# 1pathplanningzzj/pointnet_refine

Hardware: AMD Instinct MI355X
Metric: lane segments/sec (fwd+bwd) at B=4096,N=1024; HBM GB/s vs roofline (higher is better)
Workload: dtype f32 (large GEMMs: 2xfp16-split MFMA, 3 products, fp32 accumulate); 1 GPU; LineRefineNet training step (fwd + deep-supervision L1 + bwd + Adam), B=4096/GPU, N=1024, M=32, C=4; global_batch=4096, points=1024, parallelism=dp1, decoder_chunk=4096

## Files before the change

pointnet_refine_amd/csrc/prh_gemm_h2.hpp:

```cpp
#pragma once
#include "prh_gemm_s3.hpp"

namespace prh {

constexpr int H2_BK = 32;
constexpr int H2_PLANE = 256 * H2_BK * 2;
constexpr int H2_OPER = 2 * H2_PLANE;
constexpr int H2_STAGE = 2 * H2_OPER;
constexpr int H2_LDS = 2 * H2_STAGE;

__device__ __forceinline__ int h2_off(int row, int k) {
  return row * 64 + ((((k >> 3) ^ (-(row >> 2))) & 3) << 4) + ((k & 7) << 1);
}

inline size_t h2_weight_bytes(int N, int K) {
  return S3_WHDR + (size_t)((N + 255) / 256) * ((K + H2_BK - 1) / H2_BK) * H2_OPER;
}

__global__ __launch_bounds__(256) void prep_weights_h2_kernel(const float* __restrict__ W, int N,
                                                              int K, long ldw, char* __restrict__ out,
                                                              const float* __restrict__ amax) {
  const int KT = (K + H2_BK - 1) / H2_BK;
  const int NT_ = (N + 255) / 256;
  const long total = (long)NT_ * 256 * KT * 4;
  const long i = (long)blockIdx.x * blockDim.x + threadIdx.x;
  if (i >= total) return;
  const int chunk = (int)(i & 3);
  long t = i >> 2;
  const int k_tile = (int)(t % KT); t /= KT;
  const int row = (int)(t & 255);
  const int n_tile = (int)(t >> 8);
  const int n = n_tile * 256 + row;
  const float S = pow2_scale(load_amax(amax));
  float v[8];
#pragma unroll
  for (int j = 0; j < 8; ++j) {
    const int k = k_tile * H2_BK + chunk * 8 + j;
    v[j] = (n < N && k < K) ? W[(size_t)n * ldw + k] * S : 0.f;
  }
  uint4 h, l;
  split2h(v[0], v[1], h.x, l.x);
  split2h(v[2], v[3], h.y, l.y);
  split2h(v[4], v[5], h.z, l.z);
  split2h(v[6], v[7], h.w, l.w);
  char* base = out + ((size_t)n_tile * KT + k_tile) * H2_OPER + h2_off(row, chunk * 8);
  *reinterpret_cast<uint4*>(base) = h;
  *reinterpret_cast<uint4*>(base + H2_PLANE) = l;
}

template <int I0 = 0, int I1 = 8>
__device__ __forceinline__ void h2_compute(f32x4 (&acc)[8][4], const char* st, int wm, int wn, int l15,
                                           int kc) {
  f16x8 wh[4], wl[4];
#pragma unroll
  for (int j = 0; j < 4; ++j) {
    const char* q = st + H2_OPER + h2_off(wn + j * 16 + l15, kc * 8);
    wh[j] = *reinterpret_cast<const f16x8*>(q);
    wl[j] = *reinterpret_cast<const f16x8*>(q + H2_PLANE);
  }
#pragma unroll
  for (int i = I0; i < I1; ++i) {
    const char* q = st + h2_off(wm + i * 16 + l15, kc * 8);
    const f16x8 ah = *reinterpret_cast<const f16x8*>(q);
    const f16x8 al = *reinterpret_cast<const f16x8*>(q + H2_PLANE);
#pragma unroll
    for (int j = 0; j < 4; ++j) {
      acc[i][j] = __builtin_amdgcn_mfma_f32_16x16x32_f16(al, wh[j], acc[i][j], 0, 0, 0);
      acc[i][j] = __builtin_amdgcn_mfma_f32_16x16x32_f16(ah, wl[j], acc[i][j], 0, 0, 0);
      acc[i][j] = __builtin_amdgcn_mfma_f32_16x16x32_f16(ah, wh[j], acc[i][j], 0, 0, 0);
    }
  }
}

template <int PRO, int EPI, bool PP = false>
__global__ __launch_bounds__(512, 2) void gemm_nt_h2_kernel(const NTParams p,
                                                            const char* __restrict__ Wp) {
  static_assert(PRO == PRO_NONE || PRO == PRO_BNRELU || PRO == PRO_GATE1, "prologue not supported");
  extern __shared__ __attribute__((aligned(16))) char smem[];
#ifdef PRH_STAMP
  unsigned t_acc[4] = {0u, 0u, 0u, 0u};
  unsigned long long t_prev = __builtin_amdgcn_s_memtime();
#endif
  const int tid = threadIdx.x, lane = tid & 63, wave = tid >> 6;
  const int l15 = lane & 15, kc = lane >> 4;
  const int wm = (wave >> 2) * 128, wn = (wave & 3) * 64;
  const int vb = xcd_remap(blockIdx.x, gridDim.x);
  const int tile_n = vb % p.tiles_n, tile_m = vb / p.tiles_n;
  const int m0 = tile_m * 256, n0 = tile_n * 256;
  const int KT = (p.K + H2_BK - 1) / H2_BK;

  const int sc = (tid & 7) * 4;
  const int sr = tid >> 3;
  const int KP = (KT + 2) * H2_BK;
  float* coef = reinterpret_cast<float*>(smem + H2_LDS);
  const float sA = pow2_scale(load_amax(p.amaxA));
  const float unscale = 1.f / (sA * pow2_scale(load_amax(p.amaxW)));

  f32x4 acc[8][4];
#pragma unroll
  for (int i = 0; i < 8; ++i)
#pragma unroll
    for (int j = 0; j < 4; ++j)
#pragma unroll
      for (int r = 0; r < 4; ++r) acc[i][j][r] = 0.f;

  float4 ra[2][4];
  const char* wsrc = Wp + (size_t)tile_n * KT * H2_OPER + tid * 16;
  const unsigned lds0 = (unsigned)(unsigned long)((__attribute__((address_space(3))) char*)smem);
  const unsigned wdst = __builtin_amdgcn_readfirstlane(lds0 + H2_OPER + wave * 1024);
  auto dma_w = [&](int kt, int stage) {
    const char* q = wsrc + (size_t)(kt < KT ? kt : KT - 1) * H2_OPER;
#pragma unroll
    for (int pc = 0; pc < 4; ++pc) glds16(q + pc * 8192, wdst + stage * H2_STAGE + pc * 8192);
  };
  constexpr int NA = PRO == PRO_GATE1 ? 0 : 4;
  int arows = p.M - m0; arows = arows > 256 ? 256 : arows;
  const __amdgpu_buffer_rsrc_t rsA = __builtin_amdgcn_make_buffer_rsrc(
      (void*)(p.A + (size_t)m0 * p.lda), 0,
      PRO == PRO_GATE1 ? 0 : (int)(((size_t)(arows - 1) * p.lda + p.K) * 4), 0x00020000);
  int voA[4];
  float gi[4] = {0.f, 0.f, 0.f, 0.f};
#pragma unroll
  for (int j = 0; j < 4; ++j) {
    voA[j] = ((sr + 64 * j) * (int)p.lda + sc) * 4;
    if (PRO == PRO_GATE1) {
      const int row = m0 + sr + 64 * j;
      gi[j] = row < p.M ? p.A[(size_t)row * p.lda] : 0.f;
    }
  }
  auto load_tile = [&](int kt, float4 (&r)[4]) {
    if (PRO == PRO_GATE1) return;
    const int so = kt * (H2_BK * 4);
#pragma unroll
    for (int j = 0; j < 4; ++j)
      r[j] = __builtin_bit_cast(float4, __builtin_amdgcn_raw_buffer_load_b128(rsA, voA[j] + so, 0, 0));
  };
  auto store_tile = [&](int kt, char* st, const float4 (&r_)[4]) {
    const int k = kt * H2_BK + sc;
    const bool kok = k < p.K || PRO != PRO_NONE;
    float4 ka = zero4(), kb = zero4();
    if (PRO != PRO_NONE) {
      ka = *reinterpret_cast<const float4*>(coef + k);
      kb = *reinterpret_cast<const float4*>(coef + KP + k);
    }
#pragma unroll
    for (int j = 0; j < 4; ++j) {
      const int r = sr + 64 * j;
      float4 v;
      if (PRO == PRO_GATE1) v = pro_apply<PRO>(make_float4(gi[j], 0.f, 0.f, 0.f), zero4(), ka, kb, zero4());
      else v = pro_apply<PRO>(r_[j], zero4(), ka, kb, zero4());
      v.x = kok ? v.x : 0.f; v.y = kok ? v.y : 0.f; v.z = kok ? v.z : 0.f; v.w = kok ? v.w : 0.f;
      if (PRO == PRO_NONE) { v.x *= sA; v.y *= sA; v.z *= sA; v.w *= sA; }
      uint2 h, l;
      split2h(v.x, v.y, h.x, l.x);
      split2h(v.z, v.w, h.y, l.y);
      char* q = st + h2_off(r, sc);
      *reinterpret_cast<uint2*>(q) = h;
      *reinterpret_cast<uint2*>(q + H2_PLANE) = l;
    }
  };
  auto iter = [&](int kt, auto cs, auto tail) {
    constexpr int CS = decltype(cs)::value;
    constexpr bool TAIL = decltype(tail)::value;
    char* cur = smem + (kt & 1) * H2_STAGE;
    char* nxt = smem + ((kt + 1) & 1) * H2_STAGE;
    if (PRO != PRO_GATE1) {
#pragma unroll
      for (int j = 0; j < 4; ++j)
        asm volatile("" : "+v"(ra[CS][j].x), "+v"(ra[CS][j].y), "+v"(ra[CS][j].z), "+v"(ra[CS][j].w));
      __builtin_amdgcn_sched_barrier(0);
    }
    dma_w(kt + 1, (kt + 1) & 1);
    __builtin_amdgcn_sched_barrier(0);
    if (!TAIL) load_tile(kt + 2, ra[CS ^ 1]);
    __builtin_amdgcn_sched_barrier(0);
    h2_compute<0, 8>(acc, cur, wm, wn, l15, kc);
    store_tile(kt + 1, nxt, ra[CS]);
#pragma unroll
    for (int g = 0; g < 48; ++g) {
      __builtin_amdgcn_sched_group_barrier(0x008, 2, 0);
      __builtin_amdgcn_sched_group_barrier(0x002, 3, 0);
    }
    if (TAIL) asm volatile("s_waitcnt vmcnt(0)" ::: "memory");
    else asm volatile("s_waitcnt vmcnt(%0)" ::"i"(NA) : "memory");
    __syncthreads();
  };

  dma_w(0, 0);
  __builtin_amdgcn_sched_barrier(0);
  load_tile(0, ra[0]);
  load_tile(1, ra[1]);
  if (PRO != PRO_NONE) {
    for (int i = tid; i < KP; i += 512) {
      const bool in = i < p.K;
      coef[i] = in ? p.pa[i] * sA : 0.f;
      coef[KP + i] = in ? p.pb[i] * sA : 0.f;
    }
    __syncthreads();
  }
  store_tile(0, smem, ra[0]);
  asm volatile("s_waitcnt vmcnt(0)" ::: "memory");
  __syncthreads();
  PRH_TICK(0)
  int kt = 0;
  if constexpr (!PP) {
    for (; kt + 2 < KT; kt += 2) {
      iter(kt, std::integral_constant<int, 1>{}, std::false_type{});
      iter(kt + 1, std::integral_constant<int, 0>{}, std::false_type{});
    }
    if (kt < KT) iter(kt, std::integral_constant<int, 1>{}, std::true_type{});
    if (kt + 1 < KT) iter(kt + 1, std::integral_constant<int, 0>{}, std::true_type{});
  } else {
    const int wr = __builtin_amdgcn_readfirstlane(wave >> 2);
    const int aoff = h2_off(wm + l15, kc * 8);
    const int woff = H2_OPER + h2_off(wn + l15, kc * 8);
    f16x8 wh[4], wl[4], ah[2], al[2];
    auto store_pass = [&](int kt1, char* st, const float4& r_, const int j) {
      const int k = kt1 * H2_BK + sc;
      const bool kok = k < p.K || PRO != PRO_NONE;
      float4 ka = zero4(), kb = zero4();
      if (PRO != PRO_NONE) {
        ka = *reinterpret_cast<const float4*>(coef + k);
        kb = *reinterpret_cast<const float4*>(coef + KP + k);
      }
      float4 v;
      if (PRO == PRO_GATE1) v = pro_apply<PRO>(make_float4(gi[j], 0.f, 0.f, 0.f), zero4(), ka, kb, zero4());
      else v = pro_apply<PRO>(r_, zero4(), ka, kb, zero4());
      v.x = kok ? v.x : 0.f; v.y = kok ? v.y : 0.f; v.z = kok ? v.z : 0.f; v.w = kok ? v.w : 0.f;
      if (PRO == PRO_NONE) { v.x *= sA; v.y *= sA; v.z *= sA; v.w *= sA; }
      uint2 h, l;
      split2h(v.x, v.y, h.x, l.x);
      split2h(v.z, v.w, h.y, l.y);
      char* q = st + h2_off(sr + 64 * j, sc);
      *reinterpret_cast<uint2*>(q) = h;
      *reinterpret_cast<uint2*>(q + H2_PLANE) = l;
    };
    auto phase = [&](int kt_, auto mp, auto cs, auto tail) {
      constexpr int MP = decltype(mp)::value;
      constexpr int CS = decltype(cs)::value;
      constexpr bool TAIL = decltype(tail)::value;
      const char* cur = smem + (kt_ & 1) * H2_STAGE;
      char* nxt = smem + ((kt_ + 1) & 1) * H2_STAGE;
      __builtin_amdgcn_sched_barrier(0);
      if (MP == 0) {
#pragma unroll
        for (int j = 0; j < 4; ++j) {
          wh[j] = *reinterpret_cast<const f16x8*>(cur + woff + j * 1024);
          wl[j] = *reinterpret_cast<const f16x8*>(cur + woff + j * 1024 + H2_PLANE);
        }
      }
#pragma unroll
      for (int i = 0; i < 2; ++i) {
        ah[i] = *reinterpret_cast<const f16x8*>(cur + aoff + (2 * MP + i) * 1024);
        al[i] = *reinterpret_cast<const f16x8*>(cur + aoff + (2 * MP + i) * 1024 + H2_PLANE);
      }
      __builtin_amdgcn_sched_barrier(0);
      store_pass(kt_ + 1, nxt, ra[CS][MP], MP);
      __builtin_amdgcn_sched_barrier(0);
      if (MP == 0) dma_w(kt_ + 1, (kt_ + 1) & 1);
      __builtin_amdgcn_sched_barrier(0);
      if (!TAIL && PRO != PRO_GATE1)
        ra[CS ^ 1][MP] = __builtin_bit_cast(float4, __builtin_amdgcn_raw_buffer_load_b128(rsA, voA[MP] + (kt_ + 2) * (H2_BK * 4), 0, 0));
      __builtin_amdgcn_sched_barrier(0);
      if (MP == 3) {
        if (TAIL || PRO == PRO_GATE1) asm volatile("s_waitcnt vmcnt(0)" ::: "memory");
        else asm volatile("s_waitcnt vmcnt(4)" ::: "memory");
      }
      asm volatile("s_waitcnt lgkmcnt(0)" ::: "memory");
      __builtin_amdgcn_sched_barrier(0);
      __builtin_amdgcn_s_barrier();
      __builtin_amdgcn_sched_barrier(0);
      __builtin_amdgcn_s_setprio(1);
#pragma unroll
      for (int i = 0; i < 2; ++i)
#pragma unroll
        for (int j = 0; j < 4; ++j)
          acc[2 * MP + i][j] = __builtin_amdgcn_mfma_f32_16x16x32_f16(al[i], wh[j], acc[2 * MP + i][j], 0, 0, 0);
#pragma unroll
      for (int i = 0; i < 2; ++i)
#pragma unroll
        for (int j = 0; j < 4; ++j)
          acc[2 * MP + i][j] = __builtin_amdgcn_mfma_f32_16x16x32_f16(ah[i], wl[j], acc[2 * MP + i][j], 0, 0, 0);
#pragma unroll
      for (int i = 0; i < 2; ++i)
#pragma unroll
        for (int j = 0; j < 4; ++j)
          acc[2 * MP + i][j] = __builtin_amdgcn_mfma_f32_16x16x32_f16(ah[i], wh[j], acc[2 * MP + i][j], 0, 0, 0);
      __builtin_amdgcn_s_setprio(0);
      __builtin_amdgcn_sched_barrier(0);
      __builtin_amdgcn_s_barrier();
      __builtin_amdgcn_sched_barrier(0);
    };
    auto tile = [&](int kt_, auto cs, auto tail) {
      phase(kt_, std::integral_constant<int, 0>{}, cs, tail);
      phase(kt_, std::integral_constant<int, 1>{}, cs, tail);
      phase(kt_, std::integral_constant<int, 2>{}, cs, tail);
      phase(kt_, std::integral_constant<int, 3>{}, cs, tail);
    };
    if (wr == 1) __builtin_amdgcn_s_barrier();
    for (; kt + 2 < KT; kt += 2) {
      tile(kt, std::integral_constant<int, 1>{}, std::false_type{});
      tile(kt + 1, std::integral_constant<int, 0>{}, std::false_type{});
    }
    if (kt < KT) tile(kt, std::integral_constant<int, 1>{}, std::true_type{});
    if (kt + 1 < KT) tile(kt + 1, std::integral_constant<int, 0>{}, std::true_type{});
    if (wr == 0) __builtin_amdgcn_s_barrier();
  }
  asm volatile("s_waitcnt vmcnt(0)" ::: "memory");
  __syncthreads();
  PRH_TICK(1)
#pragma unroll
  for (int i = 0; i < 8; ++i)
#pragma unroll
    for (int j = 0; j < 4; ++j)
#pragma unroll
      for (int r = 0; r < 4; ++r) acc[i][j][r] *= unscale;
  nt_epilogue_vec<EPI, 4>(acc, p, m0 + wm, n0 + wn, tile_m * 2 + (wave >> 2), lane,
                          reinterpret_cast<float*>(smem) + wave * (32 * EPI_LDW));
#ifdef PRH_STAMP
  PRH_TICK(2)
  asm volatile("s_waitcnt vmcnt(0)" ::: "memory");
  PRH_TICK(3)
  const int which = (p.K == 1024 && p.N == 1984) ? 0 : (p.K == 1984 && p.N == 1024) ? 1 : (p.K == 256 && p.N == 1536) ? 2 : (p.K == 512 && p.N == 1024) ? 3 : -1;
  if (g_prh_stamp != nullptr && which >= 0 && blockIdx.x == gridDim.x / 2 + 3 && lane == 0 && (wave & 3) == 0) {
    unsigned* o = g_prh_stamp + 64 + which * 16 + (wave >> 2) * 8;
#pragma unroll
    for (int i = 0; i < 4; ++i) o[i] = t_acc[i];
    o[4] = (unsigned)KT;
  }
#endif
}

typedef __fp16 fp16x4 __attribute__((__vector_size__(4 * sizeof(__fp16))));
constexpr int TR_ROW = 576;
constexpr int TR_PLANE = 16 * TR_ROW;
constexpr int TR_OPER = 2 * TR_PLANE;
constexpr int TR_STAGE = 2 * TR_OPER;
constexpr int TR_LDS = 2 * TR_STAGE;

__device__ __forceinline__ f16x8 tr_fragment(const char* plane, int col0, int lane) {
  const int g = lane >> 4, j = lane & 15;
  const char* a = plane + ((g >> 1) * 8 + (j >> 2)) * TR_ROW + (col0 + (g & 1) * 16 + 4 * (j & 3)) * 2;
  const fp16x4 lo = __builtin_amdgcn_ds_read_tr16_b64_v4f16(
      (__attribute__((address_space(3))) fp16x4*)(a));
  const fp16x4 hi = __builtin_amdgcn_ds_read_tr16_b64_v4f16(
      (__attribute__((address_space(3))) fp16x4*)(a + 4 * TR_ROW));
  struct Pair { fp16x4 a, b; } pr = {lo, hi};
  return __builtin_bit_cast(f16x8, pr);
}

constexpr int TR_PACE = 8;
constexpr int TR_PACE_SPINS = 256;
constexpr int TR_SIDE_MAX_COLS = 4096;
inline size_t tr_side_lds(int cols) { return (size_t)3 * ((cols + 255) / 256 * 256) * 4 + 64; }
typedef unsigned int u32x4 __attribute__((ext_vector_type(4)));

template <int PROB, bool SIDE = false>
__global__ __launch_bounds__(512, 2) void gemm_tn_tr_kernel(const TNParams p) {
  static_assert(PROB == PRO_NONE || PROB == PRO_BNRELU, "prologue not supported");
  extern __shared__ __attribute__((aligned(16))) char smem[];
  const int tid = threadIdx.x, lane = tid & 63, wave = tid >> 6;
  const int wm = (wave >> 2) * 128, wn = (wave & 3) * 64;
  int b = xcd_remap(blockIdx.x, gridDim.x);
  const int tile_n = b % p.tiles_n; b /= p.tiles_n;
  const int tile_m = b % p.tiles_m; b /= p.tiles_m;
  const int split = b;
  const int m0 = tile_m * 256, n0 = tile_n * 256;
  const int p_begin = split * p.rows_per_split;
  int p_end = p_begin + p.rows_per_split;
  if (p_end > p.P) p_end = p.P;
  const int KT = (p_end - p_begin + S3_BK - 1) / S3_BK;

  const int c4 = (tid & 63) * 4, r8 = tid >> 6;
  const bool aok = (m0 + c4) < p.Mo, bok = (n0 + c4) < p.Ni;
  const float sA = pow2_scale(load_amax(p.amaxA)), sB = pow2_scale(load_amax(p.amaxB));
  const float sAm = aok ? sA : 0.f, sBm = bok ? sB : 0.f;
  float4 qa = zero4(), qb = zero4();
  if (PROB == PRO_BNRELU && bok) {
    qa = ldg4(p.qa + n0 + c4); qb = ldg4(p.qb + n0 + c4);
    qa.x *= sB; qa.y *= sB; qa.z *= sB; qa.w *= sB; qb.x *= sB; qb.y *= sB; qb.z *= sB; qb.w *= sB;
  }
  const bool want_cs = p.colsum != nullptr && tile_n == 0;

  f32x16 acc[4][2];
#pragma unroll
  for (int i = 0; i < 4; ++i)
#pragma unroll
    for (int j = 0; j < 2; ++j)
#pragma unroll
      for (int r = 0; r < 16; ++r) acc[i][j][r] = 0.f;

  const int nrows = p_end - p_begin > 0 ? p_end - p_begin : 0;
  int acols = p.Mo - m0; acols = acols > 256 ? 256 : acols;
  int bcols = p.Ni - n0; bcols = bcols > 256 ? 256 : bcols;
  const size_t abytes = nrows > 0 ? ((size_t)(nrows - 1) * p.lda + acols) * 4 : 0;
  const size_t bbytes = nrows > 0 ? ((size_t)(nrows - 1) * p.ldb + bcols) * 4 : 0;
  const __amdgpu_buffer_rsrc_t rsA = __builtin_amdgcn_make_buffer_rsrc(
      (void*)(p.A + (size_t)p_begin * p.lda + m0), 0, (int)abytes, 0x00020000);
  const __amdgpu_buffer_rsrc_t rsB = __builtin_amdgcn_make_buffer_rsrc(
      (void*)(p.B + (size_t)p_begin * p.ldb + n0), 0, (int)bbytes, 0x00020000);
  const int stepA = (int)p.lda * 4, stepB = (int)p.ldb * 4;
  const int voA = r8 * stepA + c4 * 4, voB = r8 * stepB + c4 * 4;

  float4 va[2][2], vb[2][2];
  float4 cs = zero4();
  auto load_tile = [&](int kt, float4 (&xa)[2], float4 (&xb)[2]) {
    const int oa = voA + kt * S3_BK * stepA, ob = voB + kt * S3_BK * stepB;
#pragma unroll
    for (int j = 0; j < 2; ++j) {
      xa[j] = __builtin_bit_cast(float4, __builtin_amdgcn_raw_buffer_load_b128(rsA, oa + j * 8 * stepA, 0, 0));
      xb[j] = __builtin_bit_cast(float4, __builtin_amdgcn_raw_buffer_load_b128(rsB, ob + j * 8 * stepB, 0, 0));
    }
  };
// ... 212 lines not shown
```

pointnet_refine_amd/csrc/prh_lib.hip:

```cpp
#include "../../include/pointnet_refine_hip.h"

#include <hip/hip_runtime.h>
#include <stdarg.h>
#include <stdio.h>
#include <string.h>

#include <mutex>
#include <vector>

#include <stdlib.h>

#include "prh_gemm.hpp"
#include "prh_attn.hpp"
#include "prh_attn16.hpp"
#include "prh_gemm_s3.hpp"
#include "prh_gemm_h2.hpp"
#include "prh_b16.hpp"
#include "prh_small.hpp"
#include "prh_attnfold.hpp"
#include "prh_fused.hpp"
#include "prh_context.hpp"
#include "prh_metrics.hpp"
#include "prh_drive.hpp"
#include "prh_match.hpp"
#include "prh_bev.hpp"
#include "prh_view.hpp"
#include "prh_fuse.hpp"
#include "prh_pcd.hpp"
#include "prh_kernels.hpp"

using namespace prh;

namespace {

thread_local char g_err[512] = "";

int fail(int code, const char* fmt, ...) {
  va_list ap;
  va_start(ap, fmt);
  vsnprintf(g_err, sizeof(g_err), fmt, ap);
  va_end(ap);
  return code;
}

#define HIP_TRY(expr)                                                                  \
  do {                                                                                 \
    hipError_t e_ = (expr);                                                            \
    if (e_ != hipSuccess)                                                              \
      return fail(PRH_ERR_HIP, "%s failed: %s (%s:%d)", #expr, hipGetErrorString(e_),  \
                  __FILE__, __LINE__);                                                 \
  } while (0)

#define LAUNCH_CHECK() HIP_TRY(hipGetLastError())
#define TRY_RC(x)                  \
  do {                             \
    int rc_ = (x);                 \
    if (rc_ != PRH_OK) return rc_; \
  } while (0)
#ifndef PRH_GEMM_DEFAULT
#define PRH_GEMM_DEFAULT 3
#endif

struct ProfRec { hipEvent_t e0, e1; char name[64]; double flops, bytes; };
struct Profiler {
  std::mutex mu;
  std::vector<ProfRec> recs;
  size_t used = 0;
  bool on = false;
} g_prof;

struct ProfScope {
  ProfRec* r = nullptr; hipStream_t st;
  ProfScope(const char* name, double flops, double bytes, hipStream_t s) : st(s) {
    if (!g_prof.on) return;
    std::lock_guard<std::mutex> lk(g_prof.mu);
    if (g_prof.used >= g_prof.recs.size()) return;
    r = &g_prof.recs[g_prof.used++];
    snprintf(r->name, sizeof(r->name), "%s", name);
    r->flops = flops; r->bytes = bytes;
    (void)hipEventRecord(r->e0, st);
  }
  ~ProfScope() { if (r) (void)hipEventRecord(r->e1, st); }
};

inline size_t align_up(size_t x, size_t a) { return (x + a - 1) / a * a; }
inline int cdiv(long a, long b) { return (int)((a + b - 1) / b); }

struct Arena {
  char* base; size_t size; size_t off = 0; bool ok = true;
// ... 184 lines not shown
  long maxld = p.lda > p.ldb ? p.lda : p.ldb;
  const TNPlan16 pl = tn_plan_b16(p.P, p.Mo, p.Ni, maxld);
  p.tiles_m = pl.tiles_m; p.tiles_n = pl.tiles_n; p.splits = pl.splits; p.rows_per_split = pl.rows_per_split;
  p.slab = slab;
  p.colsum = colsum_out != nullptr ? colsum_slab : nullptr;
  p.pace = nullptr;
  if (pl.tiles_m * pl.tiles_n >= 8 && pl.splits <= ABSMAX_MAX_BLOCKS && pl.rows_per_split >= 16384) {
    p.pace = reinterpret_cast<int*>(slab + (size_t)pl.splits * p.Mo * p.Ni + 64);
    if (hipMemsetAsync(p.pace, 0, sizeof(int) * pl.splits, st) != hipSuccess)
      return fail(PRH_ERR_HIP, "gemm_tn_b16: memset of the pacing counters failed");
  }
  const long blocks = (long)pl.tiles_m * pl.tiles_n * pl.splits;
  static const int attr = allow_big_lds(gemm_tn_b16_kernel<PROB>);
  if (attr != PRH_OK) return attr;
  {
    char nm[64];
    snprintf(nm, sizeof(nm), "gemm_tn_b16<0,%d> Mo=%d Ni=%d", PROB, p.Mo, p.Ni);
    const double by = 2.0 * (double)p.P * p.Mo + (PROB == PRO_GATE1 ? 4.0 * p.P : 2.0 * (double)p.P * p.Ni) + 4.0 * (double)p.Mo * p.Ni;
    ProfScope ps(nm, 2.0 * p.P * (double)p.Mo * p.Ni, by, st);
    hipLaunchKernelGGL((gemm_tn_b16_kernel<PROB>), dim3((unsigned)blocks), dim3(512), TB_LDS, st, p);
    LAUNCH_CHECK();
  }
  if (C != nullptr && colsum_out != nullptr) {
    const size_t len = (size_t)p.Mo * p.Ni + (size_t)p.Mo;
    hipLaunchKernelGGL(slab_reduce2_kernel, dim3(cdiv((long)len, 256)), dim3(256), 0, st, slab, pl.splits, p.Mo, p.Ni, C,
                       ldc, (const float*)colsum_slab, p.Mo, colsum_out);
    LAUNCH_CHECK();
    return PRH_OK;
  }
  if (C != nullptr) {
    hipLaunchKernelGGL(slab_reduce_kernel, dim3(cdiv((long)p.Mo * p.Ni, 256)), dim3(256), 0, st, slab, pl.splits, p.Mo,
                       p.Ni, C, ldc);
    LAUNCH_CHECK();
  }
  if (colsum_out != nullptr) {
    hipLaunchKernelGGL(slab_reduce_kernel, dim3(cdiv(p.Mo, 256)), dim3(256), 0, st, colsum_slab, pl.splits, 1, p.Mo,
                       colsum_out, (long)p.Mo);
    LAUNCH_CHECK();
  }
  return PRH_OK;
}

inline bool al16(const void* q) { return (reinterpret_cast<uintptr_t>(q) & 15) == 0; }
inline bool small_nt_ok(const NTParams& p, bool nn) {
  if (p.M < 1 || (p.K % SM_BK) != 0 || (p.lda & 3) || (p.ldw & 3) || !al16(p.A) || !al16(p.W)) return false;
  if ((long)cdiv(p.M, BM) * cdiv(p.N, BN) >= 192) return false;
  if (nn && (p.N & 31)) return false;
  return true;
}
template <int TM, int TN, int KS, bool NN, int EPI = EPI_BIAS>
int launch_small_cfg(NTParams& p, hipStream_t st) {
  static const int attr = allow_big_lds(gemm_small_kernel<TM, TN, KS, NN, EPI>);
  if (attr != PRH_OK) return attr;
  p.tiles_n = cdiv(p.N, TN * 32);
  const long tiles = (long)p.tiles_n * cdiv(p.M, TM * 32);
  char nm[64];
  snprintf(nm, sizeof(nm), "gemm_small<%d%d%d,%s,%d> K=%d N=%d", TM, TN, KS, NN ? "nn" : "nt", EPI, p.K, p.N);
  const double by = 4.0 * ((double)p.M * p.K + (double)p.M * p.N * ((p.flags & F_RESID) || EPI == EPI_DGRAD ? 2 : 1) + (double)p.N * p.K);
  ProfScope ps(nm, 2.0 * p.M * (double)p.N * p.K, by, st);
  hipLaunchKernelGGL((gemm_small_kernel<TM, TN, KS, NN, EPI>), dim3((unsigned)tiles), dim3(256), (small_lds<TM, TN, KS>()), st, p);
  LAUNCH_CHECK();
  return PRH_OK;
}
template <bool NN, int EPI = EPI_BIAS>
int launch_small(NTParams& p, hipStream_t st) {
  p.flags &= ~F_POOL;
  const bool n64 = !NN || (p.N & 63) == 0;
  if (n64 && (long)cdiv(p.M, 64) * cdiv(p.N, 64) >= 192) return launch_small_cfg<2, 2, 1, NN, EPI>(p, st);
  if (n64 && (long)cdiv(p.M, 32) * cdiv(p.N, 64) >= 192) return launch_small_cfg<1, 2, 2, NN, EPI>(p, st);
  return launch_small_cfg<1, 1, 4, NN, EPI>(p, st);
}
constexpr int TN_SMALL_MAX_P = 16384;
inline bool small_tn_dims_ok(int P, int Mo, int Ni) {
  return P >= 64 && P <= TN_SMALL_MAX_P && (P & 63) == 0 && (Mo & 63) == 0 && (Ni & 63) == 0;
}
inline void small_tn_plan(int P, int Mo, int Ni, int& splits, int& rps) {
  const int tiles = (Mo / 64) * (Ni / 64), chunks = P / 64;
  int s = cdiv(512, tiles);
  s = s > chunks ? chunks : (s < 1 ? 1 : s);
  rps = cdiv(chunks, s) * 64;
  splits = cdiv(P, rps);
}

template <int PRO, int EPI>
int launch_nt(Cores c, NTParams& p, hipStream_t st, StatInfo* si = nullptr) {
  if (p.M <= 0 || p.N <= 0) return PRH_OK;
  if ((p.K & 3) || (PRO != PRO_GATE1 && (p.lda & 3)) || (p.ldw & 3) ||
      (PRO == PRO_BNBWD && (p.lda2 & 3)))
    return fail(PRH_ERR_ARG, "gemm_nt: K/lda/ldw must be multiples of 4 (K=%d lda=%ld ldw=%ld)",
                p.K, p.lda, p.ldw);
  if constexpr (PRO == PRO_NONE && EPI == EPI_BIAS) {
    if (c.mode == 4 && c.core == 2 && nt_b16_generic_ok(p)) return launch_nt_b16<PRO_NONE, EPI_BIAS, false, false>(p, st, si);
  }
  const bool want_pool = (p.flags & F_POOL) != 0;
  p.flags &= ~F_POOL;
  char nm[64];
  const double by = 4.0 * ((double)p.M * p.K * (PRO == PRO_BNBWD ? 2 : (PRO == PRO_GATE1 ? 0 : 1)) +
                           (double)p.M * p.N * (EPI == EPI_GATE ? 3 : (EPI == EPI_DGRAD ? 2 : 1)) +
                           (double)p.N * p.K);
  {
    if (p.wprep != nullptr && nt_use_s3(c, p.M, p.N, p.K) && p.lda <= 65536 && p.lda2 <= 65536 &&
        !(EPI == EPI_GATE && ((p.N | (int)p.ldc | (int)p.lde1 | (int)p.ldc2) & 3) != 0)) {
      const int KT = cdiv(p.K, S3_BK), NTl = cdiv(p.N, S3_BN);
      const long th = (long)NTl * 256 * KT * 2;
      float* hdr = reinterpret_cast<float*>(p.wprep);
      const char* img = p.wprep + S3_WHDR;
      if (c.core == 3) {
        if (p.amaxW == nullptr) {
          TRY_RC((measure_absmax<PRO_NONE>(p.W, p.ldw, nullptr, 0, nullptr, nullptr, nullptr, p.N, p.K, hdr, hdr + 64, st)));
          p.amaxW = hdr;
        }
        if (p.amaxA == nullptr) {
          TRY_RC((measure_absmax<PRO>(p.A, p.lda, p.A2, p.lda2, p.pa, p.pb, p.pc, p.M, p.K, hdr + 1, hdr + 64, st)));
          p.amaxA = hdr + 1;
        }
      }
      if constexpr (PRO == PRO_NONE || PRO == PRO_BNRELU || PRO == PRO_GATE1) {
        const bool vec_ok = ((p.N | (int)p.ldc) & 3) == 0 && (p.E1 == nullptr || ((int)p.lde1 & 3) == 0) &&
                            (p.flags & F_E1_ROWVEC) == 0 && (p.C2 == nullptr || ((int)p.ldc2 & 3) == 0);
        const int KT2 = cdiv(p.K, H2_BK);
        const size_t lds = (size_t)H2_LDS + (PRO == PRO_NONE ? 0 : 2 * (size_t)(KT2 + 2) * H2_BK * 4);
        if (c.core == 3 && vec_ok && lds <= 160 * 1024) {
          const long th2 = (long)NTl * 256 * KT2 * 4;
          hipLaunchKernelGGL(prep_weights_h2_kernel, dim3((unsigned)cdiv(th2, 256)), dim3(256), 0, st, p.W,
                             p.N, p.K, p.ldw, p.wprep + S3_WHDR, p.amaxW);
          LAUNCH_CHECK();
          p.tiles_n = NTl;
          if (want_pool) p.flags |= F_POOL;
          static const int attr_h2 = allow_big_lds(gemm_nt_h2_kernel<PRO, EPI>, gemm_nt_h2_kernel<PRO, EPI, true>);
          if (attr_h2 != PRH_OK) return attr_h2;
          snprintf(nm, sizeof(nm), "gemm_nt_h2<%d,%d> K=%d N=%d", PRO, EPI, p.K, p.N);
          ProfScope ps(nm, 2.0 * p.M * (double)p.N * p.K, by, st);
          if (g_h2_pp)
            hipLaunchKernelGGL((gemm_nt_h2_kernel<PRO, EPI, true>), dim3((unsigned)(NTl * cdiv(p.M, 256))), dim3(512),
                               lds, st, p, img);
          else
            hipLaunchKernelGGL((gemm_nt_h2_kernel<PRO, EPI>), dim3((unsigned)(NTl * cdiv(p.M, 256))), dim3(512),
                               lds, st, p, img);
          LAUNCH_CHECK();
          if (si) { si->count = 2 * cdiv(p.M, S3_BM); si->rows = 128; }
          return PRH_OK;
        }
      }
      hipLaunchKernelGGL(prep_weights_s3_kernel, dim3((unsigned)cdiv(th, 256)), dim3(256), 0, st,
                         p.W, p.N, p.K, p.ldw, 0, p.wprep + S3_WHDR, c.core == 3 ? p.amaxW : nullptr);
      LAUNCH_CHECK();
      p.tiles_n = NTl;
      const long tiles = (long)NTl * cdiv(p.M, S3_BM);
      static const int attr_rc = allow_big_lds(gemm_nt_s3_kernel<PRO, EPI, 3>, gemm_nt_s3_kernel<PRO, EPI, 1>,
                                               gemm_nt_s3_kernel<PRO, EPI, 2>);
      if (attr_rc != PRH_OK) return attr_rc;
      snprintf(nm, sizeof(nm), "gemm_nt_%s<%d,%d> K=%d N=%d", c.core == 3 ? "h2g1" : c.tag(), PRO, EPI, p.K, p.N);
      ProfScope ps(nm, 2.0 * p.M * (double)p.N * p.K, by, st);
      switch (c.core) {
        case 2: launch_nt_s3<PRO, EPI, 1>(p, tiles, img, st); break;
        case 3: launch_nt_s3<PRO, EPI, 2>(p, tiles, img, st); break;
        default: launch_nt_s3<PRO, EPI, 3>(p, tiles, img, st);
      }
      LAUNCH_CHECK();
      if (si) { si->count = 2 * cdiv(p.M, S3_BM); si->rows = 128; }
      return PRH_OK;
    }
  }
  if constexpr (PRO == PRO_NONE && EPI == EPI_BIAS) {
    if (small_nt_ok(p, false)) return launch_small<false>(p, st);
  }
  p.tiles_n = cdiv(p.N, BN);
  const long tiles = (long)p.tiles_n * cdiv(p.M, BM);
  snprintf(nm, sizeof(nm), "gemm_nt<%d,%d> K=%d N=%d", PRO, EPI, p.K, p.N);
  ProfScope ps(nm, 2.0 * p.M * (double)p.N * p.K, by, st);
  if (p.N <= 64)
    hipLaunchKernelGGL((gemm_nt_kernel<PRO, EPI, true>), dim3((unsigned)tiles), dim3(256), 0, st, p);
  else
    hipLaunchKernelGGL((gemm_nt_kernel<PRO, EPI>), dim3((unsigned)tiles), dim3(256), 0, st, p);
  LAUNCH_CHECK();
  if (si) { si->count = 2 * cdiv(p.M, BM); si->rows = 64; }
  return PRH_OK;
}

constexpr int TN_S3_MAX_LD = 4096;
struct TNPlan { int tiles_m, tiles_n, splits, rows_per_split; bool s3; };
inline TNPlan tn_plan(Cores c, int P, int Mo, int Ni, bool allow_s3, long maxld = TN_S3_MAX_LD) {
  TNPlan pl;
  pl.s3 = allow_s3 && tn_use_s3(c, P, Mo, Ni);
  const int tile = pl.s3 ? 256 : 128, bk = pl.s3 ? S3_BK : BK;
  pl.tiles_m = cdiv(Mo, tile);
  pl.tiles_n = cdiv(Ni, tile);
  const int tiles = pl.tiles_m * pl.tiles_n;
  int s = cdiv(pl.s3 ? (P >= 262144 ? 768 : 256) : 1024, tiles);
  if (pl.s3) {
    int best = s; double bw = 1e9;
    for (int c = (s > 3 ? s - 2 : 1); c <= s + 4; ++c) {
      const double blocks = (double)tiles * c, w = (double)cdiv((long)blocks, 256L) * 256.0 / blocks;
      if (w < bw - 1e-3) { bw = w; best = c; }
    }
    s = best;
  }
  const int minrows = pl.s3 ? 512 : 128;
  const int smax = cdiv(P, minrows) < 1 ? 1 : cdiv(P, minrows);
  if (s > smax) s = smax;
  if (s < 1) s = 1;
  int rps = cdiv(P, s);
  rps = cdiv(rps, bk) * bk;
  if (rps < bk) rps = bk;
  const int cap = (int)((2147483647L / (4L * (maxld < 4 ? 4 : maxld))) / bk * bk);
  if (pl.s3 && rps > cap) rps = cap;
  pl.splits = cdiv(P, rps) < 1 ? 1 : cdiv(P, rps);
  pl.rows_per_split = rps;
  return pl;
}
constexpr int TN_HDR = S3_HDR_FLOATS;
inline size_t tn_splits_bound(Cores cores, int P, int Mo, int Ni) {
  const size_t a = (size_t)tn_plan(cores, P, Mo, Ni, true).splits, b = (size_t)tn_plan(cores, P, Mo, Ni, false).splits;
  size_t c = (size_t)tn_plan(cores, P, Mo, Ni, true, 4).splits;
  if (small_tn_dims_ok(P, Mo, Ni)) {
// ... 2673 lines not shown
```

Measured before the change: 9685 segments/s.

## Make h2 GEMM persistent for short-K plain operands, prefetching next tile during epilogue

```diff
diff --git a/pointnet_refine_amd/csrc/prh_gemm_h2.hpp b/pointnet_refine_amd/csrc/prh_gemm_h2.hpp
--- a/pointnet_refine_amd/csrc/prh_gemm_h2.hpp
+++ b/pointnet_refine_amd/csrc/prh_gemm_h2.hpp
@@ -8,6 +8,9 @@
 constexpr int H2_OPER = 2 * H2_PLANE;
 constexpr int H2_STAGE = 2 * H2_OPER;
 constexpr int H2_LDS = 2 * H2_STAGE;
+constexpr int H2_WALK_LDS = H2_STAGE + 8 * 32 * EPI_LDW * 4;
+static_assert(H2_WALK_LDS >= H2_LDS && H2_WALK_LDS <= 160 * 1024, "walk: stages and scratch-at-stage-1 inside the LDS");
+template <int EPI> constexpr bool H2_WALK_PF2 = EPI == EPI_BIAS;
 
 __device__ __forceinline__ int h2_off(int row, int k) {
   return row * 64 + ((((k >> 3) ^ (-(row >> 2))) & 3) << 4) + ((k & 7) << 1);
@@ -72,62 +75,75 @@
   }
 }
 
-template <int PRO, int EPI, bool PP = false>
+template <int PRO, int EPI, bool PP = false, bool WALK = false>
 __global__ __launch_bounds__(512, 2) void gemm_nt_h2_kernel(const NTParams p,
                                                             const char* __restrict__ Wp) {
   static_assert(PRO == PRO_NONE || PRO == PRO_BNRELU || PRO == PRO_GATE1, "prologue not supported");
+  static_assert(!WALK || (PRO == PRO_NONE && !PP), "the tile walk serves plain operands on the one-barrier k-loop");
   extern __shared__ __attribute__((aligned(16))) char smem[];
 #ifdef PRH_STAMP
   unsigned t_acc[4] = {0u, 0u, 0u, 0u};
   unsigned long long t_prev = __builtin_amdgcn_s_memtime();
 #endif
-  const int tid = threadIdx.x, lane = tid & 63, wave = tid >> 6;
-  const int l15 = lane & 15, kc = lane >> 4;
-  const int wm = (wave >> 2) * 128, wn = (wave & 3) * 64;
-  const int vb = xcd_remap(blockIdx.x, gridDim.x);
-  const int tile_n = vb % p.tiles_n, tile_m = vb / p.tiles_n;
-  const int m0 = tile_m * 256, n0 = tile_n * 256;
+  int lane, wave, l15, kc, wm, wn, sc, sr;
+  auto lanes = [&]() {
+    int tid = threadIdx.x;
+    if (WALK) asm volatile("" : "+v"(tid));
+    lane = tid & 63; wave = tid >> 6;
+    l15 = lane & 15; kc = lane >> 4;
+    wm = (wave >> 2) * 128; wn = (wave & 3) * 64;
+    sc = (tid & 7) * 4;
+    sr = tid >> 3;
+    return tid;
+  };
+  const int ntiles = p.tiles_n * ((p.M + 255) / 256);
+  int tbase = 0;
+  auto tile_id = [&]() {
+    const int left = ntiles - tbase;
+    return tbase + xcd_remap(blockIdx.x, left < (int)gridDim.x ? left : (int)gridDim.x);
+  };
+  int tile_n, tile_m, m0, n0;
   const int KT = (p.K + H2_BK - 1) / H2_BK;
 
-  const int sc = (tid & 7) * 4;
-  const int sr = tid >> 3;
   const int KP = (KT + 2) * H2_BK;
   float* coef = reinterpret_cast<float*>(smem + H2_LDS);
   const float sA = pow2_scale(load_amax(p.amaxA));
   const float unscale = 1.f / (sA * pow2_scale(load_amax(p.amaxW)));
 
   f32x4 acc[8][4];
-#pragma unroll
-  for (int i = 0; i < 8; ++i)
-#pragma unroll
-    for (int j = 0; j < 4; ++j)
-#pragma unroll
-      for (int r = 0; r < 4; ++r) acc[i][j][r] = 0.f;
 
   float4 ra[2][4];
-  const char* wsrc = Wp + (size_t)tile_n * KT * H2_OPER + tid * 16;
+  const char* wsrc;
   const unsigned lds0 = (unsigned)(unsigned long)((__attribute__((address_space(3))) char*)smem);
-  const unsigned wdst = __builtin_amdgcn_readfirstlane(lds0 + H2_OPER + wave * 1024);
+  unsigned wdst;
   auto dma_w = [&](int kt, int stage) {
     const char* q = wsrc + (size_t)(kt < KT ? kt : KT - 1) * H2_OPER;
 #pragma unroll
     for (int pc = 0; pc < 4; ++pc) glds16(q + pc * 8192, wdst + stage * H2_STAGE + pc * 8192);
   };
   constexpr int NA = PRO == PRO_GATE1 ? 0 : 4;
-  int arows = p.M - m0; arows = arows > 256 ? 256 : arows;
-  const __amdgpu_buffer_rsrc_t rsA = __builtin_amdgcn_make_buffer_rsrc(
-      (void*)(p.A + (size_t)m0 * p.lda), 0,
-      PRO == PRO_GATE1 ? 0 : (int)(((size_t)(arows - 1) * p.lda + p.K) * 4), 0x00020000);
+  __amdgpu_buffer_rsrc_t rsA;
   int voA[4];
   float gi[4] = {0.f, 0.f, 0.f, 0.f};
-#pragma unroll
-  for (int j = 0; j < 4; ++j) {
-    voA[j] = ((sr + 64 * j) * (int)p.lda + sc) * 4;
-    if (PRO == PRO_GATE1) {
-      const int row = m0 + sr + 64 * j;
-      gi[j] = row < p.M ? p.A[(size_t)row * p.lda] : 0.f;
-    }
-  }
+  auto enter_tile = [&](int vb) {
+    const int tid = lanes();
+    tile_n = vb % p.tiles_n; tile_m = vb / p.tiles_n;
+    m0 = tile_m * 256; n0 = tile_n * 256;
+    wsrc = Wp + (size_t)tile_n * KT * H2_OPER + tid * 16;
+    wdst = __builtin_amdgcn_readfirstlane(lds0 + H2_OPER + wave * 1024);
+    int arows = p.M - m0; arows = arows > 256 ? 256 : arows;
+    rsA = __builtin_amdgcn_make_buffer_rsrc(
+        (void*)(p.A + (size_t)m0 * p.lda), 0,
+        PRO == PRO_GATE1 ? 0 : (int)(((size_t)(arows - 1) * p.lda + p.K) * 4), 0x00020000);
+#pragma unroll
+    for (int j = 0; j < 4; ++j) {
+      voA[j] = ((sr + 64 * j) * (int)p.lda + sc) * 4;
+      if (PRO == PRO_GATE1) {
+        const int row = m0 + sr + 64 * j;
+        gi[j] = row < p.M ? p.A[(size_t)row * p.lda] : 0.f;
+      }
+    }
+  };
   auto load_tile = [&](int kt, float4 (&r)[4]) {
     if (PRO == PRO_GATE1) return;
     const int so = kt * (H2_BK * 4);
@@ -186,149 +202,187 @@
     __syncthreads();
   };
 
+  enter_tile(tile_id());
   dma_w(0, 0);
   __builtin_amdgcn_sched_barrier(0);
   load_tile(0, ra[0]);
   load_tile(1, ra[1]);
   if (PRO != PRO_NONE) {
-    for (int i = tid; i < KP; i += 512) {
+    for (int i = threadIdx.x; i < KP; i += 512) {
       const bool in = i < p.K;
       coef[i] = in ? p.pa[i] * sA : 0.f;
       coef[KP + i] = in ? p.pb[i] * sA : 0.f;
     }
     __syncthreads();
   }
-  store_tile(0, smem, ra[0]);
-  asm volatile("s_waitcnt vmcnt(0)" ::: "memory");
-  __syncthreads();
-  PRH_TICK(0)
-  int kt = 0;
-  if constexpr (!PP) {
-    for (; kt + 2 < KT; kt += 2) {
-      iter(kt, std::integral_constant<int, 1>{}, std::false_type{});
-      iter(kt + 1, std::integral_constant<int, 0>{}, std::false_type{});
-    }
-    if (kt < KT) iter(kt, std::integral_constant<int, 1>{}, std::true_type{});
-    if (kt + 1 < KT) iter(kt + 1, std::integral_constant<int, 0>{}, std::true_type{});
-  } else {
-    const int wr = __builtin_amdgcn_readfirstlane(wave >> 2);
-    const int aoff = h2_off(wm + l15, kc * 8);
-    const int woff = H2_OPER + h2_off(wn + l15, kc * 8);
-    f16x8 wh[4], wl[4], ah[2], al[2];
-    auto store_pass = [&](int kt1, char* st, const float4& r_, const int j) {
-      const int k = kt1 * H2_BK + sc;
-      const bool kok = k < p.K || PRO != PRO_NONE;
-      float4 ka = zero4(), kb = zero4();
-      if (PRO != PRO_NONE) {
-        ka = *reinterpret_cast<const float4*>(coef + k);
-        kb = *reinterpret_cast<const float4*>(coef + KP + k);
-      }
-      float4 v;
-      if (PRO == PRO_GATE1) v = pro_apply<PRO>(make_float4(gi[j], 0.f, 0.f, 0.f), zero4(), ka, kb, zero4());
-      else v = pro_apply<PRO>(r_, zero4(), ka, kb, zero4());
-      v.x = kok ? v.x : 0.f; v.y = kok ? v.y : 0.f; v.z = kok ? v.z : 0.f; v.w = kok ? v.w : 0.f;
-      if (PRO == PRO_NONE) { v.x *= sA; v.y *= sA; v.z *= sA; v.w *= sA; }
-      uint2 h, l;
-      split2h(v.x, v.y, h.x, l.x);
-      split2h(v.z, v.w, h.y, l.y);
-      char* q = st + h2_off(sr + 64 * j, sc);
-      *reinterpret_cast<uint2*>(q) = h;
-      *reinterpret_cast<uint2*>(q + H2_PLANE) = l;
-    };
-    auto phase = [&](int kt_, auto mp, auto cs, auto tail) {
-      constexpr int MP = decltype(mp)::value;
-      constexpr int CS = decltype(cs)::value;
-      constexpr bool TAIL = decltype(tail)::value;
-      const char* cur = smem + (kt_ & 1) * H2_STAGE;
-      char* nxt = smem + ((kt_ + 1) & 1) * H2_STAGE;
-      __builtin_amdgcn_sched_barrier(0);
-      if (MP == 0) {
-#pragma unroll
-        for (int j = 0; j < 4; ++j) {
-          wh[j] = *reinterpret_cast<const f16x8*>(cur + woff + j * 1024);
-          wl[j] = *reinterpret_cast<const f16x8*>(cur + woff + j * 1024 + H2_PLANE);
+  for (;;) {
+#pragma unroll
+    for (int i = 0; i < 8; ++i)
+#pragma unroll
+      for (int j = 0; j < 4; ++j)
+#pragma unroll
+        for (int r = 0; r < 4; ++r) acc[i][j][r] = 0.f;
+    store_tile(0, smem, ra[0]);
+    asm volatile("s_waitcnt vmcnt(0)" ::: "memory");
+    __syncthreads();
+    PRH_TICK(0)
+    int kt = 0;
+    if constexpr (!PP) {
+      for (; kt + 2 < KT; kt += 2) {
+        iter(kt, std::integral_constant<int, 1>{}, std::false_type{});
+        iter(kt + 1, std::integral_constant<int, 0>{}, std::false_type{});
+      }
+      if (kt < KT) iter(kt, std::integral_constant<int, 1>{}, std::true_type{});
+      if (kt + 1 < KT) iter(kt + 1, std::integral_constant<int, 0>{}, std::true_type{});
+    } else {
+      const int wr = __builtin_amdgcn_readfirstlane(wave >> 2);
+      const int aoff = h2_off(wm + l15, kc * 8);
+      const int woff = H2_OPER + h2_off(wn + l15, kc * 8);
+      f16x8 wh[4], wl[4], ah[2], al[2];
+      auto store_pass = [&](int kt1, char* st, const float4& r_, const int j) {
+        const int k = kt1 * H2_BK + sc;
+        const bool kok = k < p.K || PRO != PRO_NONE;
+        float4 ka = zero4(), kb = zero4();
+        if (PRO != PRO_NONE) {
+          ka = *reinterpret_cast<const float4*>(coef + k);
+          kb = *reinterpret_cast<const float4*>(coef + KP + k);
         }
-      }
-#pragma unroll
-      for (int i = 0; i < 2; ++i) {
-        ah[i] = *reinterpret_cast<const f16x8*>(cur + aoff + (2 * MP + i) * 1024);
-        al[i] = *reinterpret_cast<const f16x8*>(cur + aoff + (2 * MP + i) * 1024 + H2_PLANE);
-      }
-      __builtin_amdgcn_sched_barrier(0);
-      store_pass(kt_ + 1, nxt, ra[CS][MP], MP);
-      __builtin_amdgcn_sched_barrier(0);
-      if (MP == 0) dma_w(kt_ + 1, (kt_ + 1) & 1);
-      __builtin_amdgcn_sched_barrier(0);
-      if (!TAIL && PRO != PRO_GATE1)
-        ra[CS ^ 1][MP] = __builtin_bit_cast(float4, __builtin_amdgcn_raw_buffer_load_b128(rsA, voA[MP] + (kt_ + 2) * (H2_BK * 4), 0, 0));
-      __builtin_amdgcn_sched_barrier(0);
-      if (MP == 3) {
-        if (TAIL || PRO == PRO_GATE1) asm volatile("s_waitcnt vmcnt(0)" ::: "memory");
-        else asm volatile("s_waitcnt vmcnt(4)" ::: "memory");
-      }
-      asm volatile("s_waitcnt lgkmcnt(0)" ::: "memory");
-      __builtin_amdgcn_sched_barrier(0);
-      __builtin_amdgcn_s_barrier();
-      __builtin_amdgcn_sched_barrier(0);
-      __builtin_amdgcn_s_setprio(1);
-#pragma unroll
-      for (int i = 0; i < 2; ++i)
-#pragma unroll
-        for (int j = 0; j < 4; ++j)
-          acc[2 * MP + i][j] = __builtin_amdgcn_mfma_f32_16x16x32_f16(al[i], wh[j], acc[2 * MP + i][j], 0, 0, 0);
-#pragma unroll
-      for (int i = 0; i < 2; ++i)
-#pragma unroll
-        for (int j = 0; j < 4; ++j)
-          acc[2 * MP + i][j] = __builtin_amdgcn_mfma_f32_16x16x32_f16(ah[i], wl[j], acc[2 * MP + i][j], 0, 0, 0);
-#pragma unroll
-      for (int i = 0; i < 2; ++i)
-#pragma unroll
-        for (int j = 0; j < 4; ++j)
-          acc[2 * MP + i][j] = __builtin_amdgcn_mfma_f32_16x16x32_f16(ah[i], wh[j], acc[2 * MP + i][j], 0, 0, 0);
-      __builtin_amdgcn_s_setprio(0);
-      __builtin_amdgcn_sched_barrier(0);
-      __builtin_amdgcn_s_barrier();
-      __builtin_amdgcn_sched_barrier(0);
-    };
-    auto tile = [&](int kt_, auto cs, auto tail) {
-      phase(kt_, std::integral_constant<int, 0>{}, cs, tail);
-      phase(kt_, std::integral_constant<int, 1>{}, cs, tail);
-      phase(kt_, std::integral_constant<int, 2>{}, cs, tail);
-      phase(kt_, std::integral_constant<int, 3>{}, cs, tail);
-    };
-    if (wr == 1) __builtin_amdgcn_s_barrier();
-    for (; kt + 2 < KT; kt += 2) {
-      tile(kt, std::integral_constant<int, 1>{}, std::false_type{});
-      tile(kt + 1, std::integral_constant<int, 0>{}, std::false_type{});
-    }
-    if (kt < KT) tile(kt, std::integral_constant<int, 1>{}, std::true_type{});
-    if (kt + 1 < KT) tile(kt + 1, std::integral_constant<int, 0>{}, std::true_type{});
-    if (wr == 0) __builtin_amdgcn_s_barrier();
-  }
-  asm volatile("s_waitcnt vmcnt(0)" ::: "memory");
-  __syncthreads();
-  PRH_TICK(1)
-#pragma unroll
-  for (int i = 0; i < 8; ++i)
-#pragma unroll
-    for (int j = 0; j < 4; ++j)
-#pragma unroll
-      for (int r = 0; r < 4; ++r) acc[i][j][r] *= unscale;
-  nt_epilogue_vec<EPI, 4>(acc, p, m0 + wm, n0 + wn, tile_m * 2 + (wave >> 2), lane,
-                          reinterpret_cast<float*>(smem) + wave * (32 * EPI_LDW));
+        float4 v;
+        if (PRO == PRO_GATE1) v = pro_apply<PRO>(make_float4(gi[j], 0.f, 0.f, 0.f), zero4(), ka, kb, zero4());
+        else v = pro_apply<PRO>(r_, zero4(), ka, kb, zero4());
+        v.x = kok ? v.x : 0.f; v.y = kok ? v.y : 0.f; v.z = kok ? v.z : 0.f; v.w = kok ? v.w : 0.f;
+        if (PRO == PRO_NONE) { v.x *= sA; v.y *= sA; v.z *= sA; v.w *= sA; }
+        uint2 h, l;
+        split2h(v.x, v.y, h.x, l.x);
+        split2h(v.z, v.w, h.y, l.y);
+        char* q = st + h2_off(sr + 64 * j, sc);
+        *reinterpret_cast<uint2*>(q) = h;
+        *reinterpret_cast<uint2*>(q + H2_PLANE) = l;
+      };
+      auto phase = [&](int kt_, auto mp, auto cs, auto tail) {
+        constexpr int MP = decltype(mp)::value;
+        constexpr int CS = decltype(cs)::value;
+        constexpr bool TAIL = decltype(tail)::value;
+        const char* cur = smem + (kt_ & 1) * H2_STAGE;
+        char* nxt = smem + ((kt_ + 1) & 1) * H2_STAGE;
+        __builtin_amdgcn_sched_barrier(0);
+        if (MP == 0) {
+#pragma unroll
+          for (int j = 0; j < 4; ++j) {
+            wh[j] = *reinterpret_cast<const f16x8*>(cur + woff + j * 1024);
+            wl[j] = *reinterpret_cast<const f16x8*>(cur + woff + j * 1024 + H2_PLANE);
+          }
+        }
+#pragma unroll
+        for (int i = 0; i < 2; ++i) {
+          ah[i] = *reinterpret_cast<const f16x8*>(cur + aoff + (2 * MP + i) * 1024);
+          al[i] = *reinterpret_cast<const f16x8*>(cur + aoff + (2 * MP + i) * 1024 + H2_PLANE);
+        }
+        __builtin_amdgcn_sched_barrier(0);
+        store_pass(kt_ + 1, nxt, ra[CS][MP], MP);
+        __builtin_amdgcn_sched_barrier(0);
+        if (MP == 0) dma_w(kt_ + 1, (kt_ + 1) & 1);
+        __builtin_amdgcn_sched_barrier(0);
+        if (!TAIL && PRO != PRO_GATE1)
+          ra[CS ^ 1][MP] = __builtin_bit_cast(float4, __builtin_amdgcn_raw_buffer_load_b128(rsA, voA[MP] + (kt_ + 2) * (H2_BK * 4), 0, 0));
+        __builtin_amdgcn_sched_barrier(0);
+        if (MP == 3) {
+          if (TAIL || PRO == PRO_GATE1) asm volatile("s_waitcnt vmcnt(0)" ::: "memory");
+          else asm volatile("s_waitcnt vmcnt(4)" ::: "memory");
+        }
+        asm volatile("s_waitcnt lgkmcnt(0)" ::: "memory");
+        __builtin_amdgcn_sched_barrier(0);
+        __builtin_amdgcn_s_barrier();
+        __builtin_amdgcn_sched_barrier(0);
+        __builtin_amdgcn_s_setprio(1);
+#pragma unroll
+        for (int i = 0; i < 2; ++i)
+#pragma unroll
+          for (int j = 0; j < 4; ++j)
+            acc[2 * MP + i][j] = __builtin_amdgcn_mfma_f32_16x16x32_f16(al[i], wh[j], acc[2 * MP + i][j], 0, 0, 0);
+#pragma unroll
+        for (int i = 0; i < 2; ++i)
+#pragma unroll
+          for (int j = 0; j < 4; ++j)
+            acc[2 * MP + i][j] = __builtin_amdgcn_mfma_f32_16x16x32_f16(ah[i], wl[j], acc[2 * MP + i][j], 0, 0, 0);
+#pragma unroll
+        for (int i = 0; i < 2; ++i)
+#pragma unroll
+          for (int j = 0; j < 4; ++j)
+            acc[2 * MP + i][j] = __builtin_amdgcn_mfma_f32_16x16x32_f16(ah[i], wh[j], acc[2 * MP + i][j], 0, 0, 0);
+        __builtin_amdgcn_s_setprio(0);
+        __builtin_amdgcn_sched_barrier(0);
+        __builtin_amdgcn_s_barrier();
+        __builtin_amdgcn_sched_barrier(0);
+      };
+      auto tile = [&](int kt_, auto cs, auto tail) {
+        phase(kt_, std::integral_constant<int, 0>{}, cs, tail);
+        phase(kt_, std::integral_constant<int, 1>{}, cs, tail);
+        phase(kt_, std::integral_constant<int, 2>{}, cs, tail);
+        phase(kt_, std::integral_constant<int, 3>{}, cs, tail);
+      };
+      if (wr == 1) __builtin_amdgcn_s_barrier();
+      for (; kt + 2 < KT; kt += 2) {
+        tile(kt, std::integral_constant<int, 1>{}, std::false_type{});
+        tile(kt + 1, std::integral_constant<int, 0>{}, std::false_type{});
+      }
+      if (kt < KT) tile(kt, std::integral_constant<int, 1>{}, std::true_type{});
+      if (kt + 1 < KT) tile(kt + 1, std::integral_constant<int, 0>{}, std::true_type{});
+      if (wr == 0) __builtin_amdgcn_s_barrier();
+    }
+    asm volatile("s_waitcnt vmcnt(0)" ::: "memory");
+    __syncthreads();
+    PRH_TICK(1)
+#pragma unroll
+    for (int i = 0; i < 8; ++i)
+#pragma unroll
+      for (int j = 0; j < 4; ++j)
+#pragma unroll
+        for (int r = 0; r < 4; ++r) acc[i][j][r] *= unscale;
+    bool more = false;
+    if constexpr (WALK) {
+      tbase += (int)gridDim.x;
+      more = (int)blockIdx.x < ntiles - tbase;
+      if (more) {
+        const int vb = tile_id();
+        int tid = threadIdx.x;
+        asm volatile("" : "+v"(tid));
+        const int tn = vb % p.tiles_n, mn = (vb / p.tiles_n) * 256;
+        const char* q = Wp + (size_t)tn * KT * H2_OPER + tid * 16;
+        const unsigned d = __builtin_amdgcn_readfirstlane(lds0 + H2_OPER + (tid >> 6) * 1024);
+#pragma unroll
+        for (int pc = 0; pc < 4; ++pc) glds16(q + pc * 8192, d + pc * 8192);
+        __builtin_amdgcn_sched_barrier(0);
+        int arows = p.M - mn; arows = arows > 256 ? 256 : arows;
+        const __amdgpu_buffer_rsrc_t rn = __builtin_amdgcn_make_buffer_rsrc(
+            (void*)(p.A + (size_t)mn * p.lda), 0, (int)(((size_t)(arows - 1) * p.lda + p.K) * 4), 0x00020000);
+#pragma unroll
+        for (int k1 = 0; k1 < (H2_WALK_PF2<EPI> ? 2 : 1); ++k1)
+#pragma unroll
+          for (int j = 0; j < 4; ++j)
+            ra[k1][j] = __builtin_bit_cast(float4, __builtin_amdgcn_raw_buffer_load_b128(
+                rn, (((tid >> 3) + 64 * j) * (int)p.lda + (tid & 7) * 4) * 4 + k1 * (H2_BK * 4), 0, 0));
+        __builtin_amdgcn_sched_barrier(0);
+      }
+    }
+    nt_epilogue_vec<EPI, 4>(acc, p, m0 + wm, n0 + wn, tile_m * 2 + (wave >> 2), lane,
+                            reinterpret_cast<float*>(smem + (WALK ? H2_STAGE : 0)) + wave * (32 * EPI_LDW));
 #ifdef PRH_STAMP
-  PRH_TICK(2)
-  asm volatile("s_waitcnt vmcnt(0)" ::: "memory");
-  PRH_TICK(3)
-  const int which = (p.K == 1024 && p.N == 1984) ? 0 : (p.K == 1984 && p.N == 1024) ? 1 : (p.K == 256 && p.N == 1536) ? 2 : (p.K == 512 && p.N == 1024) ? 3 : -1;
-  if (g_prh_stamp != nullptr && which >= 0 && blockIdx.x == gridDim.x / 2 + 3 && lane == 0 && (wave & 3) == 0) {
-    unsigned* o = g_prh_stamp + 64 + which * 16 + (wave >> 2) * 8;
-#pragma unroll
-    for (int i = 0; i < 4; ++i) o[i] = t_acc[i];
-    o[4] = (unsigned)KT;
-  }
+    PRH_TICK(2)
+    asm volatile("s_waitcnt vmcnt(0)" ::: "memory");
+    PRH_TICK(3)
+    const int which = (p.K == 1024 && p.N == 1984) ? 0 : (p.K == 1984 && p.N == 1024) ? 1 : (p.K == 256 && p.N == 1536) ? 2 : (p.K == 512 && p.N == 1024) ? 3 : -1;
+    if (g_prh_stamp != nullptr && which >= 0 && blockIdx.x == gridDim.x / 2 + 3 && lane == 0 && (wave & 3) == 0) {
+      unsigned* o = g_prh_stamp + 64 + which * 16 + (wave >> 2) * 8;
+#pragma unroll
+      for (int i = 0; i < 4; ++i) o[i] = t_acc[i];
+      o[4] = (unsigned)KT;
+    }
 #endif
+    if (!WALK || !more) break;
+    enter_tile(tile_id());
+    if (!H2_WALK_PF2<EPI>) load_tile(1, ra[1]);
+  }
 }
 
 typedef __fp16 fp16x4 __attribute__((__vector_size__(4 * sizeof(__fp16))));
diff --git a/pointnet_refine_amd/csrc/prh_lib.hip b/pointnet_refine_amd/csrc/prh_lib.hip
--- a/pointnet_refine_amd/csrc/prh_lib.hip
+++ b/pointnet_refine_amd/csrc/prh_lib.hip
@@ -5,6 +5,7 @@
 #include <stdio.h>
 #include <string.h>
 
+#include <atomic>
 #include <mutex>
 #include <vector>
 
@@ -355,6 +356,26 @@
   splits = cdiv(P, rps);
 }
 
+template <int EPI>
+int h2_walk_resident(int* out) {
+  constexpr int MAX_DEV = 64;
+  static std::atomic<int> cache[MAX_DEV];
+  int dev = 0;
+  HIP_TRY(hipGetDevice(&dev));
+  int r = (dev >= 0 && dev < MAX_DEV) ? cache[dev].load(std::memory_order_relaxed) : 0;
+  if (r == 0) {
+    static const int attr = allow_big_lds(gemm_nt_h2_kernel<PRO_NONE, EPI, false, true>);
+    if (attr != PRH_OK) return attr;
+    int per_cu = 0, cus = 0;
+    HIP_TRY(hipOccupancyMaxActiveBlocksPerMultiprocessor(&per_cu, gemm_nt_h2_kernel<PRO_NONE, EPI, false, true>, 512, H2_WALK_LDS));
+    HIP_TRY(hipDeviceGetAttribute(&cus, hipDeviceAttributeMultiprocessorCount, dev));
+    if (per_cu <= 0 || cus <= 0) return fail(PRH_ERR_HIP, "gemm_nt_h2: no resident workgroup at %d B of LDS", H2_WALK_LDS);
+    r = per_cu * cus;
+    if (dev >= 0 && dev < MAX_DEV) cache[dev].store(r, std::memory_order_relaxed);
+  }
+  *out = r;
+  return PRH_OK;
+}
 template <int PRO, int EPI>
 int launch_nt(Cores c, NTParams& p, hipStream_t st, StatInfo* si = nullptr) {
   if (p.M <= 0 || p.N <= 0) return PRH_OK;
@@ -404,6 +425,18 @@
           if (attr_h2 != PRH_OK) return attr_h2;
           snprintf(nm, sizeof(nm), "gemm_nt_h2<%d,%d> K=%d N=%d", PRO, EPI, p.K, p.N);
           ProfScope ps(nm, 2.0 * p.M * (double)p.N * p.K, by, st);
+          if constexpr (PRO == PRO_NONE) {
+            if (!g_h2_pp && p.K <= 512) {
+              int resident = 0;
+              TRY_RC((h2_walk_resident<EPI>(&resident)));
+              const long tiles = (long)NTl * cdiv(p.M, 256);
+              hipLaunchKernelGGL((gemm_nt_h2_kernel<PRO_NONE, EPI, false, true>), dim3((unsigned)(tiles < resident ? tiles : resident)),
+                                 dim3(512), H2_WALK_LDS, st, p, img);
+              LAUNCH_CHECK();
+              if (si) { si->count = 2 * cdiv(p.M, S3_BM); si->rows = 128; }
+              return PRH_OK;
+            }
+          }
           if (g_h2_pp)
             hipLaunchKernelGGL((gemm_nt_h2_kernel<PRO, EPI, true>), dim3((unsigned)(NTl * cdiv(p.M, 256))), dim3(512),
                                lds, st, p, img);
```

After: 9742 segments/s (median of 6 runs). About the same (+0.6%).
